# microsoft/hyperspace

Hardware: AMD Instinct MI355X
Metric: index-build GB/s + indexed filter/join query latency (s), 1/2/4/8 MI355X (higher is better)
Workload: dtype int64/fp64 columnar; 1 GPU; model=covering-index(key,val) build + filter + co-bucketed join, num_buckets=200, parallelism=bucket-parallel dp1, RCCL all-to-all exchange, device=cuda

## Files before the change

hyperspace_amd/csrc/binding.cpp:

```cpp

#include <torch/extension.h>

#include <c10/hip/HIPStream.h>

#include <algorithm>
#include <tuple>
#include <vector>

#include "kernels/kernels.h"

namespace {

hipStream_t current_stream() {
  return c10::hip::getCurrentHIPStream().stream();
}

void check_cuda(const torch::Tensor& t, const char* name) {
  TORCH_CHECK(t.is_cuda(), name, " must be a device tensor");
  TORCH_CHECK(t.is_contiguous(), name, " must be contiguous");
}

int normalize_dtype_code(torch::ScalarType t) {
  switch (t) {
    case torch::kInt64: return 0;
    case torch::kInt32: return 1;
    case torch::kFloat64: return 2;
    case torch::kFloat32: return 3;
    case torch::kInt16: return 4;
    case torch::kInt8: return 5;
    case torch::kBool: return 6;
    default:
      TORCH_CHECK(false, "unsupported sort-key dtype");
  }
}

torch::Tensor murmur3_bucket(std::vector<torch::Tensor> keys,
                             int64_t num_buckets,
                             std::vector<torch::Tensor> masks = {}) {
  TORCH_CHECK(!keys.empty(), "need at least one key column");
  TORCH_CHECK(masks.empty() || masks.size() == keys.size(),
              "masks must be empty or parallel to keys");
  TORCH_CHECK(num_buckets > 0 && num_buckets <= (int64_t)INT32_MAX,
              "murmur3_bucket: num_buckets must be in 1..INT32_MAX, got ",
              num_buckets);
  auto n = keys[0].numel();
  auto dev = keys[0].device();
  torch::Tensor h;
  if (keys.size() > 1)
    h = torch::empty({n}, torch::dtype(torch::kInt32).device(dev));
  auto out = torch::empty({n}, torch::dtype(torch::kInt32).device(dev));
  auto stream = current_stream();
  bool first = true;
  for (size_t ci = 0; ci < keys.size(); ++ci) {
    auto& k = keys[ci];
    check_cuda(k, "key");
    TORCH_CHECK(k.numel() == n, "key column length mismatch");
    torch::Tensor col = k;
    int kind;
    switch (col.scalar_type()) {
      case torch::kInt64:
        kind = 1;
        break;
      case torch::kFloat64:
        kind = 3;
        break;
      case torch::kInt32:
        kind = 0;
        break;
      case torch::kFloat32:
        kind = 2;
        break;
      case torch::kInt16:
      case torch::kInt8:
      case torch::kBool:
        col = col.to(torch::kInt32);
        kind = 0;
        break;
      default:
        TORCH_CHECK(false, "unsupported hash-key dtype");
    }
    const uint8_t* valid = nullptr;
    torch::Tensor mcol;
    if (!masks.empty() && masks[ci].numel() > 0) {
      mcol = masks[ci];
      check_cuda(mcol, "mask");
      TORCH_CHECK(mcol.numel() == n, "mask length mismatch");
      TORCH_CHECK(mcol.scalar_type() == torch::kBool ||
                      mcol.scalar_type() == torch::kUInt8,
                  "mask must be bool/uint8");
      valid = (const uint8_t*)mcol.data_ptr();
    }
// ... 659 lines not shown
                      masks[c].scalar_type() == torch::kUInt8,
                  "mask must be bool/uint8");
      held.push_back(aligned16(masks[c]));
      mptr[c] = (const uint8_t*)held.back().data_ptr();
    }
  }
  auto stream = current_stream();
  int64_t tile = hsk::group_tile_size();
  int64_t n_tiles = (n + tile - 1) / tile;
  auto tile_counts = torch::empty({n_tiles}, opts);
  hsk::group_offsets_count(kptr, mptr, (int)keys.size(), n,
                           tile_counts.data_ptr<int64_t>(), stream);
  auto tile_offsets = torch::empty({n_tiles}, opts);
  auto total = torch::empty({1}, opts);
  hsk::exclusive_scan_i64(tile_counts.data_ptr<int64_t>(),
                          tile_offsets.data_ptr<int64_t>(), n_tiles,
                          total.data_ptr<int64_t>(), stream);
  int64_t n_groups = total.cpu().item<int64_t>();
  auto out = torch::empty({n_groups + 1}, opts);
  hsk::group_offsets_emit(kptr, mptr, (int)keys.size(), n,
                          tile_offsets.data_ptr<int64_t>(),
                          total.data_ptr<int64_t>(), out.data_ptr<int64_t>(),
                          stream);
  return out;
}

std::vector<torch::Tensor> segmented_reduce(torch::Tensor values,
                                            torch::Tensor valid,
                                            torch::Tensor offsets,
                                            int64_t want) {
  check_cuda(values, "values");
  int dtype;
  switch (values.scalar_type()) {
    case torch::kInt64: dtype = 0; break;
    case torch::kInt32: dtype = 1; break;
    case torch::kFloat64: dtype = 2; break;
    case torch::kFloat32: dtype = 3; break;
    default:
      TORCH_CHECK(false, "segmented_reduce: values must be int32, int64, "
                         "float32 or float64");
  }
  bool is_float = dtype >= 2;
  auto dev = values.device();
  int64_t n = values.numel();
  auto off_d = offsets.to(dev, torch::kInt64).contiguous();
  TORCH_CHECK(off_d.numel() >= 1, "offsets must have n_groups + 1 entries");
  int64_t n_groups = off_d.numel() - 1;
  auto i64 = torch::dtype(torch::kInt64).device(dev);
  auto sum_opts = is_float ? torch::dtype(torch::kFloat64).device(dev) : i64;
  auto sums = torch::zeros({(want & 1) ? n_groups : 0}, sum_opts);
  auto mins = torch::zeros({(want & 2) ? n_groups : 0}, values.options());
  auto maxs = torch::zeros({(want & 4) ? n_groups : 0}, values.options());
  auto counts = torch::zeros({n_groups}, i64);
  if (n == 0 || n_groups == 0) return {sums, mins, maxs, counts};
  values = aligned16(values);
  const uint8_t* vptr = nullptr;
  if (valid.numel() > 0) {
    check_cuda(valid, "valid");
    TORCH_CHECK(valid.numel() == n, "valid length mismatch");
    TORCH_CHECK(valid.scalar_type() == torch::kBool ||
                    valid.scalar_type() == torch::kUInt8,
                "valid must be bool/uint8");
    valid = aligned16(valid);
    vptr = (const uint8_t*)valid.data_ptr();
  }
  int64_t tile = hsk::group_tile_size();
  int64_t n_tiles = (n + tile - 1) / tile;
  auto tile_groups = torch::empty({n_tiles + 1}, i64);
  auto partials =
      torch::empty({4 * hsk::segmented_reduce_num_blocks(n)}, i64);
  hsk::segmented_reduce(values.data_ptr(), dtype, vptr,
                        off_d.data_ptr<int64_t>(), n, n_groups,
                        (want & 1) ? sums.data_ptr() : nullptr,
                        (want & 2) ? mins.data_ptr() : nullptr,
                        (want & 4) ? maxs.data_ptr() : nullptr,
                        counts.data_ptr<int64_t>(),
                        tile_groups.data_ptr<int64_t>(),
                        partials.data_ptr<int64_t>(), current_stream());
  return {sums, mins, maxs, counts};
}

int64_t group_tile_size() { return hsk::group_tile_size(); }

}

torch::Tensor select_range_u64_pub(torch::Tensor keys, int64_t lo,
                                   int64_t hi, bool lo_incl, bool hi_incl) {
  TORCH_CHECK(keys.is_cuda() && keys.is_contiguous(), "keys");
  auto n = keys.numel();
  auto opts = torch::dtype(torch::kInt64).device(keys.device());
  if (n == 0) return torch::empty({0}, opts);
  auto stream = c10::hip::getCurrentHIPStream().stream();
  int64_t nb = hsk::select_num_blocks(n);
  auto bcounts = torch::empty({nb}, opts);
  auto total = torch::empty({1}, opts);
  uint64_t ulo = (uint64_t)lo;
  uint64_t uhi = (uint64_t)hi;
  hsk::select_range_count((const uint64_t*)keys.data_ptr<int64_t>(), n, ulo,
                          uhi, lo_incl, hi_incl,
                          bcounts.data_ptr<int64_t>(),
                          total.data_ptr<int64_t>(), stream);
  int64_t n_out = total.cpu().item<int64_t>();
  auto out = torch::empty({n_out}, opts);
  if (n_out > 0) {
    hsk::select_range_emit((const uint64_t*)keys.data_ptr<int64_t>(), n, ulo,
                           uhi, lo_incl, hi_incl,
                           bcounts.data_ptr<int64_t>(),
                           out.data_ptr<int64_t>(), stream);
  }
  return out;
}

PYBIND11_MODULE(TORCH_EXTENSION_NAME, m) {
  m.def("murmur3_bucket", &murmur3_bucket, "Spark-compatible murmur3 bucket",
        py::arg("keys"), py::arg("num_buckets"),
        py::arg("masks") = std::vector<torch::Tensor>{});
  m.def("normalize_key", &normalize_key, "order-preserving u64 key",
        py::arg("vals"), py::arg("canonical") = false);
  m.def("radix_sort_pairs", &radix_sort_pairs, "stable LSD radix sort");
  m.def("radix_sort_plan", &radix_sort_plan,
        "pass plan of the radix sort for a varying-bit mask: "
        "(radix, [shifts])");
  m.def("exclusive_scan", &exclusive_scan,
        "device-wide exclusive scan of an int64 tensor: (out, total)");
  m.def("merge_join", &merge_join, "segmented sorted merge join",
        py::arg("lkeys"), py::arg("rkeys"), py::arg("lseg"), py::arg("rseg"),
        py::arg("mode") = 0);
  m.def("select_range_u64", &select_range_u64_pub, "range filter compaction");
  m.def("isin_sorted", &isin_sorted, "sorted-set membership");
  m.def("segmented_minmax", &segmented_minmax, "per-segment min/max");
  m.def("bloom_build", &bloom_build, "bloom filter build");
  m.def("bloom_probe", &bloom_probe, "bloom filter probe");
  m.def("bloom_probe_many", &bloom_probe_many,
        "K9 device sketch-predicate probe over per-file filters");
  m.def("zorder_key", &zorder_key, "z-order bit interleave");
  m.def("gather_rows", &gather_rows,
        "row gather by an int64 or int32 index");
  m.def("bucket_sort_perm", &bucket_sort_perm,
        "fused (bucket, integer key) sort: (perm int32, sorted key column, "
        "seg) or None when the key range is too wide");
  m.def("copy_unaligned", &copy_unaligned,
        "device parquet page decode (unaligned copy)");
  m.def("run_merge_perm", &run_merge_perm,
        "segmented two-sorted-run merge permutation");
  m.def("group_offsets", &group_offsets,
        "offsets of adjacent equal-key runs: int64 [n_groups + 1]",
        py::arg("keys"), py::arg("masks") = std::vector<torch::Tensor>{});
  m.def("segmented_reduce", &segmented_reduce,
        "fused per-group (sum, min, max, count); want bits 1/2/4");
  m.def("group_tile_size", &group_tile_size,
        "rows per tile of the group-by kernels");
  m.def("snappy_decompress", &snappy_decompress,
        "device snappy raw-block page decompression; returns status");
  m.def("decode_def_levels", &decode_def_levels,
        "host RLE-hybrid def-level decode -> bool validity");
  m.def("parse_rle_runs_batch", &parse_rle_runs_batch,
        py::call_guard<py::gil_scoped_release>(),
        "batched RLE-hybrid run parse over many pages");
  m.def("parse_rle_runs", &parse_rle_runs,
        py::call_guard<py::gil_scoped_release>(),
        "host parse of an RLE/bit-packed hybrid run table");
  m.def("parse_byte_arrays", &parse_byte_arrays,
        py::call_guard<py::gil_scoped_release>(),
        "host PLAIN byte-array page parse -> (offsets, bytes)");
  m.def("host_memcpy", &host_memcpy,
        "GIL-released buffer -> cpu-u8-tensor memcpy");
  m.def("rle_decode", &rle_decode,
        "device RLE/bit-packed dictionary-index decode");
}
```

hyperspace_amd/index/covering/index.py:

```python

from __future__ import annotations

import os
from typing import Any, Dict, List, Optional, Tuple

import torch

from ..base import Index, IndexerContext
from ...config import IndexConstants
from ...exceptions import HyperspaceException
from ...log.entry import (Schema, register_derived_dataset,
                          COVERING_INDEX_TYPE)
from ... import ops
from ...execution.columnar import ColumnBatch, StringColumn
from ...sources.parquet_io import (bucket_file_name, write_batch_parquet,
                                   read_files_batch, bucket_id_of_file)


class CoveringIndex(Index):
    def __init__(self, indexed_columns: List[str],
                 included_columns: List[str], schema: Schema,
                 num_buckets: int, properties: Dict[str, str]):
        self.indexed_columns = list(indexed_columns)
        self.included_columns = list(included_columns)
        self.schema = schema
        self.num_buckets = num_buckets
        self._properties = dict(properties)

    @property
    def kind(self) -> str:
        return "CoveringIndex"

    @property
    def kind_abbr(self) -> str:
        return "CI"

    def indexed_columns_list(self) -> List[str]:
        return list(self.indexed_columns)

    def referenced_columns(self) -> List[str]:
        return self.indexed_columns + self.included_columns

    @property
    def can_handle_deleted_files(self) -> bool:
        return (self._properties.get(IndexConstants.LINEAGE_PROPERTY, "false")
                .lower() == "true")

    @property
    def has_lineage(self) -> bool:
        return self.can_handle_deleted_files

    def with_new_properties(self, props: Dict[str, str]) -> "CoveringIndex":
        return CoveringIndex(self.indexed_columns, self.included_columns,
                             self.schema, self.num_buckets, props)

    def to_json(self) -> Dict[str, Any]:
        return {
            "type": COVERING_INDEX_TYPE,
            "indexedColumns": self.indexed_columns,
            "includedColumns": self.included_columns,
            "schema": self.schema.to_json(),
            "numBuckets": self.num_buckets,
            "properties": self._properties,
        }

    @staticmethod
    def from_json(d: Dict[str, Any]) -> "CoveringIndex":
        return CoveringIndex(
            d["indexedColumns"], d["includedColumns"],
            Schema.from_json(d["schema"]), d["numBuckets"],
            d.get("properties", {}))

    def write(self, ctx: IndexerContext, index_data) -> List[str]:
        from ...execution.scan_stream import ScanStream
        os.makedirs(ctx.index_data_path, exist_ok=True)

        import torch.distributed as dist
        distributed = dist.is_available() and dist.is_initialized() and \
            dist.get_world_size() > 1
        task_id = dist.get_rank() if distributed else 0

        if isinstance(index_data, ScanStream):
            batches = index_data.batches()
            n_groups = len(index_data.file_groups())
        else:
# ... 253 lines not shown
                "includedColumns": self.included_columns,
                "numBuckets": self.num_buckets}



def _multi_key_sort_perm(batch: ColumnBatch, key_cols: List[str]
                         ) -> torch.Tensor:
    n = batch.num_rows
    dev = batch.device
    perm = torch.arange(n, dtype=torch.int64, device=dev)
    for c in reversed(key_cols):
        keys = ops.sql_key(batch.tensor(c))[perm]
        _, perm = ops.sort_pairs(keys, perm)
        m = batch.mask(c)
        if m is not None and not bool(m.all()):
            f = m[perm]
            perm = perm[torch.cat([
                torch.nonzero(~f, as_tuple=False).flatten(),
                torch.nonzero(f, as_tuple=False).flatten()])]
    return perm


def _bucket_seg_offsets(sorted_bkeys_u64: torch.Tensor, num_buckets: int
                        ) -> torch.Tensor:
    probes = ops.cpu_ref.normalize_key(
        torch.arange(num_buckets + 1, dtype=torch.int64)).to(
            sorted_bkeys_u64.device)
    if sorted_bkeys_u64.numel() and int(sorted_bkeys_u64.max()) >= 0 \
            and int(sorted_bkeys_u64.min()) >= 0:
        seg = torch.searchsorted(
            sorted_bkeys_u64,
            torch.arange(num_buckets + 1, dtype=torch.int64,
                         device=sorted_bkeys_u64.device))
        return seg.cpu()
    sortable = sorted_bkeys_u64 ^ (-0x8000000000000000)
    sortable_probes = probes ^ (-0x8000000000000000)
    return torch.searchsorted(sortable, sortable_probes).cpu()


def _fused_bucket_sort(batch: ColumnBatch, bucket_ids: torch.Tensor,
                       key_cols: List[str], num_buckets: int
                       ) -> Optional[Tuple[ColumnBatch, torch.Tensor]]:
    if len(key_cols) != 1 or os.environ.get("HS_FUSED_BUCKET_SORT") == "0":
        return None
    key_name = batch._stored_key(key_cols[0])
    key = batch.columns[key_name]
    if isinstance(key, StringColumn) or batch.has_nulls(key_name):
        return None
    res = ops.bucket_sort_perm(key, bucket_ids, num_buckets)
    if res is None:
        return None
    perm, sorted_key, seg = res
    cols: Dict[str, Any] = {}
    for k, v in batch.columns.items():
        if k == key_name:
            cols[k] = sorted_key
        elif isinstance(v, StringColumn):
            cols[k] = StringColumn(ops.gather_rows(v.codes, perm), v.values)
        else:
            cols[k] = ops.gather_rows(v, perm)
    return ColumnBatch(
        cols, {k: m[perm] for k, m in batch.masks.items()}), seg


def sort_by_bucket_and_keys(batch: ColumnBatch, bucket_ids: torch.Tensor,
                            key_cols: List[str], num_buckets: int
                            ) -> Tuple[ColumnBatch, torch.Tensor]:
    fused = _fused_bucket_sort(batch, bucket_ids, key_cols, num_buckets)
    if fused is not None:
        return fused
    perm = _multi_key_sort_perm(batch, key_cols)
    b64 = ops.gather_rows(bucket_ids.to(torch.int64), perm)
    sorted_bkeys, perm2 = ops.sort_pairs(ops.normalize_key(b64), perm)
    batch = batch.gather(perm2)
    probes = ops.cpu_ref.normalize_key(
        torch.arange(num_buckets + 1, dtype=torch.int64)).to(
            sorted_bkeys.device)
    sortable = sorted_bkeys ^ (-0x8000000000000000)
    sortable_probes = probes ^ (-0x8000000000000000)
    seg = torch.searchsorted(sortable, sortable_probes).cpu()
    return batch, seg


def write_bucketed(batch: ColumnBatch, seg: torch.Tensor, out_dir: str,
                   num_buckets: int, task_id: int = 0,
                   after_event: Optional["torch.cuda.Event"] = None
                   ) -> List[str]:
    from concurrent.futures import ThreadPoolExecutor
    from ...execution.columnar import StringColumn
    from ...sources.parquet_io import _pinned_get, _pinned_put
    on_device = batch.device.type == "cuda"
    if on_device and os.environ.get("HS_WRITE_V2"):
        if after_event is not None:
            torch.cuda.current_stream().wait_event(after_event)
        host_cols = {}
        host_masks = {}
        held_bufs = []
        for name, col in batch.columns.items():
            if isinstance(col, StringColumn):
                host_cols[name] = col.to("cpu")
                continue
            nb = col.numel() * col.element_size()
            bufp = _pinned_get(nb)
            host = bufp[:nb].view(col.dtype)
            host.copy_(col, non_blocking=True)
            host_cols[name] = host
            held_bufs.append(bufp)
        for name, m in batch.masks.items():
            host_masks[name] = m.to("cpu")
        torch.cuda.current_stream().synchronize()
        host_batch = ColumnBatch(host_cols, host_masks)
        out = write_bucketed(host_batch, seg, out_dir, num_buckets,
                             task_id)
        for bufp in held_bufs:
            _pinned_put(bufp)
        return out
    jobs = []
    for b in range(num_buckets):
        lo, hi = int(seg[b]), int(seg[b + 1])
        if hi <= lo:
            continue
        jobs.append((b, lo, hi,
                     os.path.join(out_dir, bucket_file_name(task_id, b))))

    streams = ([torch.cuda.Stream(device=batch.device)
                for _ in range(min(8, max(1, len(jobs))))]
               if on_device else [])

    def write_one(job_i):
        b, lo, hi, out = jobs[job_i]
        piece = batch.slice(lo, hi)
        held = []
        if on_device:
            s = streams[job_i % len(streams)]
            if after_event is not None:
                s.wait_event(after_event)
            cols = {}
            masks = {}
            with torch.cuda.stream(s):
                for name, col in piece.columns.items():
                    if isinstance(col, StringColumn):
                        cols[name] = col.to("cpu")
                        continue
                    nb = col.numel() * col.element_size()
                    bufp = _pinned_get(nb)
                    host = bufp[:nb].view(col.dtype)
                    host.copy_(col, non_blocking=True)
                    cols[name] = host
                    held.append(bufp)
                for name, m in piece.masks.items():
                    masks[name] = m.to("cpu")
            s.synchronize()
            piece = ColumnBatch(cols, masks)
        write_batch_parquet(piece, out)
        for bufp in held:
            _pinned_put(bufp)
        return out

    if len(jobs) <= 2:
        return [write_one(i) for i in range(len(jobs))]
    with ThreadPoolExecutor(max_workers=16) as pool:
        return list(pool.map(write_one, range(len(jobs))))


register_derived_dataset(COVERING_INDEX_TYPE, CoveringIndex)
```

hyperspace_amd/rules/score_optimizer.py:

```python

from __future__ import annotations

from typing import Dict, List, Tuple

from .candidate_collector import Candidate
from .filter_reason import ReasonCollector
from .hyperspace_rules import (AggregateIndexRule, FilterIndexRule,
                               HyperspaceRule, JoinIndexRule, NoOpRule)
from ..plan.nodes import LogicalPlan


class ScoreBasedIndexPlanOptimizer:
    def __init__(self, session, reasons: ReasonCollector):
        self.session = session
        self.reasons = reasons
        self.rules: List[HyperspaceRule] = [
            FilterIndexRule(session, reasons),
            JoinIndexRule(session, reasons),
            AggregateIndexRule(session, reasons),
        ]
        try:
            from ..index.zorder.rule import ZOrderFilterIndexRule
            self.rules.append(ZOrderFilterIndexRule(session, reasons))
        except ImportError:
            pass
        try:
            from ..index.dataskipping.rule import ApplyDataSkippingIndex
            self.rules.append(ApplyDataSkippingIndex(session, reasons))
        except ImportError:
            pass
        self.rules.append(NoOpRule(session, reasons))

    def apply(self, plan: LogicalPlan,
              candidates: Dict[int, List[Candidate]]) -> LogicalPlan:
        best, _ = self._rec_apply(plan, candidates, {})
        return best

    def _rec_apply(self, plan: LogicalPlan, candidates,
                   memo: Dict[int, Tuple[LogicalPlan, float]]
                   ) -> Tuple[LogicalPlan, float]:
        key = id(plan)
        if key in memo:
            return memo[key]
        best_plan, best_score = plan, -1.0
        for rule in self.rules:
            transformed, score = rule.apply(plan, candidates)
            if transformed is plan and rule.name != "NoOpRule" and \
                    score == 0.0:
                continue
            child_results = [self._rec_apply(c, candidates, memo)
                             for c in transformed.children]
            total = score + sum(s for _, s in child_results)
            if transformed is not plan or rule.name == "NoOpRule":
                candidate_plan = (
                    transformed.with_children([p for p, _ in child_results])
                    if child_results else transformed)
                if total > best_score:
                    best_plan, best_score = candidate_plan, total
        memo[key] = (best_plan, max(best_score, 0.0))
        return memo[key]
```

hyperspace_amd/sources/native_parquet.py:

```python

from __future__ import annotations

import os
import struct
from typing import Any, Dict, List, NamedTuple, Optional, Tuple

import numpy as np

MAGIC = b"PAR1"

T_INT32, T_INT64, T_FLOAT, T_DOUBLE, T_BYTE_ARRAY = 1, 2, 4, 5, 6
_NP_TO_PARQUET = {
    np.dtype("int64"): T_INT64,
    np.dtype("int32"): T_INT32,
    np.dtype("float64"): T_DOUBLE,
    np.dtype("float32"): T_FLOAT,
}
_PARQUET_TO_NP = {v: k for k, v in _NP_TO_PARQUET.items()}

ENC_PLAIN = 0
ENC_PLAIN_DICTIONARY = 2
ENC_RLE = 3
ENC_RLE_DICTIONARY = 8
CODEC_UNCOMPRESSED = 0
# ... 170 lines not shown
    w.field_i32(2, nbytes)
    w.field_i32(3, nbytes)
    w.field_struct_begin(5)
    w.field_i32(1, num_values)
    w.field_i32(2, encoding)
    w.field_i32(3, ENC_RLE if has_def_levels else ENC_PLAIN)
    w.field_i32(4, ENC_PLAIN)
    w.struct_end()
    w.struct_end()
    return bytes(w.buf)


def _dict_page_header(num_values: int, nbytes: int) -> bytes:
    w = TWriter()
    w.struct_begin()
    w.field_i32(1, PAGE_DICTIONARY)
    w.field_i32(2, nbytes)
    w.field_i32(3, nbytes)
    w.field_struct_begin(7)
    w.field_i32(1, num_values)
    w.field_i32(2, ENC_PLAIN_DICTIONARY)
    w.struct_end()
    w.struct_end()
    return bytes(w.buf)


def _bitpack(vals: np.ndarray, width: int) -> bytes:
    n = len(vals)
    pad = (-n) % 8
    if pad:
        vals = np.concatenate(
            [vals, np.zeros(pad, dtype=vals.dtype)])
    bits = ((vals[:, None].astype(np.uint64)
             >> np.arange(width, dtype=np.uint64)) & 1).astype(np.uint8)
    return np.packbits(bits.reshape(-1), bitorder="little").tobytes()


def _dict_indices_payload(codes: np.ndarray, num_dict: int) -> Tuple[
        bytes, int]:
    bw = max(1, (num_dict - 1).bit_length()) if num_dict > 1 else 1
    groups = (len(codes) + 7) // 8
    body = _varint((groups << 1) | 1) + _bitpack(codes, bw)
    return bytes([bw]) + body, bw


def _plain_byte_array_dict(values: List[str]) -> bytes:
    out = bytearray()
    for v in values:
        b = v.encode("utf-8")
        out += struct.pack("<I", len(b))
        out += b
    return bytes(out)


def _statistics(arr: np.ndarray) -> Tuple[bytes, bytes]:
    return arr.min().tobytes(), arr.max().tobytes()


def _def_levels_payload(mask: np.ndarray) -> bytes:
    groups = (len(mask) + 7) // 8
    packed = np.packbits(mask.astype(np.uint8), bitorder="little")
    body = _varint((groups << 1) | 1) + packed.tobytes()
    return struct.pack("<I", len(body)) + body


_LAYOUT_CACHE: "Dict[str, Tuple[Tuple[int, int], int, list]]" = {}
_LAYOUT_CACHE_MAX = 16384


def layout_cache_get(path: str):
    ent = _LAYOUT_CACHE.get(path)
    if ent is None:
        return None
    try:
        st = os.stat(path)
    except OSError:
        return None
    if ent[0] != (st.st_size, st.st_mtime_ns):
        _LAYOUT_CACHE.pop(path, None)
        return None
    return ent[1], ent[2]


def _layout_cache_put(path: str, num_rows: int, layouts: list) -> None:
    if len(_LAYOUT_CACHE) >= _LAYOUT_CACHE_MAX:
        for k in list(_LAYOUT_CACHE)[:_LAYOUT_CACHE_MAX // 8]:
            _LAYOUT_CACHE.pop(k, None)
    st = os.stat(path)
    _LAYOUT_CACHE[path] = ((st.st_size, st.st_mtime_ns), num_rows, layouts)


def write_parquet_native(columns: "Dict[str, np.ndarray]", path: str,
                         masks: "Optional[Dict[str, np.ndarray]]" = None
                         ) -> Tuple[int, int]:
    names = list(columns.keys())
    arrays: List[Any] = []
    for n in names:
        c = columns[n]
        arrays.append(c if isinstance(c, StrCol)
                      else np.ascontiguousarray(c))
    num_rows = len(arrays[0]) if arrays else 0
    col_masks: List[Optional[np.ndarray]] = []
    for n, a in zip(names, arrays):
        if not isinstance(a, StrCol) and a.dtype not in _NP_TO_PARQUET:
            raise ValueError(f"dtype {a.dtype} not supported natively")
        assert len(a) == num_rows
        m = (masks or {}).get(n)
        if m is not None and bool(m.all()):
            m = None
        col_masks.append(m)

    chunks: List[Any] = []
    col_meta: List[Tuple] = []
    layouts: List[ColumnChunkLayout] = []
    offset = 4
    for name, arr, mask in zip(names, arrays, col_masks):
        if isinstance(arr, StrCol):
            dict_payload = _plain_byte_array_dict(arr.values)
            dict_header = _dict_page_header(len(arr.values),
                                            len(dict_payload))
            dict_off = offset
            offset += len(dict_header) + len(dict_payload)
            chunks.append(dict_header)
            chunks.append(dict_payload)

            codes = arr.codes if mask is None else arr.codes[mask]
            null_count = int(num_rows - len(codes))
            idx_payload, bw = _dict_indices_payload(codes,
                                                    len(arr.values))
            lvl_len = 0
            if mask is None:
                payload: Any = idx_payload
            else:
                levels = _def_levels_payload(mask)
                lvl_len = len(levels)
                payload = levels + idx_payload
            header = _page_header(num_rows, len(payload), mask is not None,
                                  encoding=ENC_PLAIN_DICTIONARY)
            col_meta.append((name, T_BYTE_ARRAY, offset,
                             offset - dict_off + len(header) + len(payload),
                             num_rows, b"", b"", null_count,
                             mask is not None, dict_off))
            layouts.append(ColumnChunkLayout(
                name, np.dtype("int32"),
                [Page("dict", offset + len(header) + lvl_len + 1,
                      offset + len(header) + len(payload), num_rows, bw)],
                num_rows, "dict",
                DictPage(dict_off + len(dict_header), offset,
                         len(arr.values)), [mask],
                is_string=True, str_values=list(arr.values)))
            chunks.append(header)
            chunks.append(payload)
            offset += len(header) + len(payload)
            continue
        lvl_len = 0
        if mask is None:
            payload = arr.data.cast("B")
            null_count = 0
            valid = arr
        else:
            valid = arr[mask]
            levels = _def_levels_payload(mask)
            lvl_len = len(levels)
            payload = levels + valid.tobytes()
            null_count = int(num_rows - len(valid))
        nbytes = len(payload)
        header = _page_header(num_rows, nbytes, mask is not None)
        mn, mx = _statistics(valid) if len(valid) else (b"", b"")
        col_meta.append((name, _NP_TO_PARQUET[arr.dtype], offset,
                         len(header) + nbytes, num_rows, mn, mx,
                         null_count, mask is not None, None))
        layouts.append(ColumnChunkLayout(
# ... 631 lines not shown
```

setup.py:

```python

import os

from setuptools import setup

os.environ.setdefault("PYTORCH_ROCM_ARCH", "gfx950")

from torch.utils.cpp_extension import BuildExtension, CUDAExtension

ROOT = os.path.dirname(os.path.abspath(__file__))

setup(
    name="hyperspace_amd",
    version="0.1.0",
    description="MI355X-native covering-index acceleration engine",
    packages=["hyperspace_amd"],
    ext_modules=[
        CUDAExtension(
            name="hyperspace_amd._hip",
            sources=[
                "hyperspace_amd/csrc/binding.cpp",
                "hyperspace_amd/csrc/kernels/kernels.hip",
                "hyperspace_amd/csrc/kernels/aggregate.hip",
            ],
            include_dirs=[os.path.join(ROOT, "hyperspace_amd", "csrc")],
            extra_compile_args={
                "cxx": ["-O3", "-std=c++17"],
                "nvcc": ["-O3", "-std=c++17"],
            },
        )
    ],
    cmdclass={"build_ext": BuildExtension},
)
```

Measured before the change: 16.66 GB/s.

## Write bucket files natively via chunked D2H pinned ring and threaded pwrite

Adds a C++ bucket writer that streams device columns in chunks through a pinned host ring on two HIP streams. A pool of writer threads pwrites each chunk straight to its offset in the parquet file, and the footer is encoded in C++. Per-bucket min/max statistics are computed on the device with segmented_reduce, and the file layout cache is filled from the fstat results, so there is no extra os.stat per file. The aim is to overlap device-to-host copies with file I/O and to drop the per-file Python write overhead. In exchange it adds a large native code path with its own parquet encoding, threading and error handling, and it removes the HS_WRITE_V2 path.

```diff
diff --git a/hyperspace_amd/csrc/binding.cpp b/hyperspace_amd/csrc/binding.cpp
--- a/hyperspace_amd/csrc/binding.cpp
+++ b/hyperspace_amd/csrc/binding.cpp
@@ -4,9 +4,11 @@
 #include <c10/hip/HIPStream.h>
 
 #include <algorithm>
+#include <string>
 #include <tuple>
 #include <vector>
 
+#include "bucket_writer.h"
 #include "kernels/kernels.h"
 
 namespace {
@@ -832,6 +834,107 @@
 
 int64_t group_tile_size() { return hsk::group_tile_size(); }
 
+std::tuple<std::vector<int64_t>, std::vector<int64_t>, std::vector<int64_t>,
+           std::vector<int64_t>>
+write_bucket_files(std::vector<torch::Tensor> cols,
+                   std::vector<std::string> names,
+                   std::vector<std::string> paths,
+                   std::vector<int64_t> row_lo, std::vector<int64_t> row_hi,
+                   std::vector<std::string> mins,
+                   std::vector<std::string> maxs, torch::Tensor ring,
+                   int64_t chunk_bytes, int64_t writer_threads,
+                   int64_t stream0, int64_t stream1, bool timing) {
+  TORCH_CHECK(!cols.empty() && cols.size() == names.size(),
+              "write_bucket_files: columns and names must be parallel");
+  TORCH_CHECK(paths.size() == row_lo.size() && paths.size() == row_hi.size(),
+              "write_bucket_files: paths and row ranges must be parallel");
+  TORCH_CHECK(mins.size() == paths.size() * cols.size() &&
+                  maxs.size() == mins.size(),
+              "write_bucket_files: one (min, max) per file and column");
+  TORCH_CHECK(chunk_bytes > 0 && writer_threads >= 1 && writer_threads <= 15,
+              "write_bucket_files: chunk_bytes > 0, 1 <= threads <= 15");
+  const bool on_device = cols[0].is_cuda();
+  const int64_t n = cols[0].numel();
+  std::vector<hsw::Column> wc;
+  for (size_t c = 0; c < cols.size(); c++) {
+    const torch::Tensor& t = cols[c];
+    TORCH_CHECK(t.dim() == 1 && t.is_contiguous() && t.numel() == n &&
+                    t.device() == cols[0].device(),
+                "write_bucket_files: columns must be 1-D, contiguous, of "
+                "one length and on one device");
+    int ptype;
+    switch (t.scalar_type()) {
+      case torch::kInt64: ptype = hsw::T_INT64; break;
+      case torch::kInt32: ptype = hsw::T_INT32; break;
+      case torch::kFloat64: ptype = hsw::T_DOUBLE; break;
+      case torch::kFloat32: ptype = hsw::T_FLOAT; break;
+      default:
+        TORCH_CHECK(false, "write_bucket_files: unsupported column dtype");
+    }
+    wc.push_back({t.data_ptr(), (int)t.element_size(), ptype, names[c]});
+  }
+  std::vector<hsw::FileJob> jobs;
+  for (size_t f = 0; f < paths.size(); f++) {
+    TORCH_CHECK(0 <= row_lo[f] && row_lo[f] < row_hi[f] && row_hi[f] <= n,
+                "write_bucket_files: row range of file ", f,
+                " is empty or outside the batch");
+    jobs.push_back({paths[f], row_lo[f], row_hi[f]});
+  }
+  std::vector<std::pair<std::string, std::string>> stats;
+  for (size_t i = 0; i < mins.size(); i++)
+    stats.emplace_back(std::move(mins[i]), std::move(maxs[i]));
+
+  hsw::Options opt;
+  opt.chunk_bytes = (size_t)chunk_bytes;
+  opt.writer_threads = (int)writer_threads;
+  opt.device_source = on_device;
+  opt.timing = timing;
+  std::vector<hsw::FileResult> res;
+  if (on_device) {
+    TORCH_CHECK(ring.device().is_cpu() && ring.is_pinned() &&
+                    ring.is_contiguous() &&
+                    ring.scalar_type() == torch::kUInt8 &&
+                    ring.numel() >= chunk_bytes,
+                "write_bucket_files: ring must be a pinned uint8 tensor of "
+                "at least one chunk");
+    opt.streams[0] = reinterpret_cast<hipStream_t>(stream0);
+    opt.streams[1] = reinterpret_cast<hipStream_t>(stream1);
+    opt.ring = ring.data_ptr();
+    opt.ring_bytes = (size_t)ring.numel();
+    hipEvent_t start = nullptr;
+    TORCH_CHECK(hipEventCreateWithFlags(&start, hipEventDisableTiming) ==
+                    hipSuccess,
+                "write_bucket_files: hipEventCreate failed");
+    hipError_t e = hipEventRecord(start, current_stream());
+    opt.start_event = start;
+    std::string err;
+    if (e != hipSuccess) {
+      err = std::string("hipEventRecord: ") + hipGetErrorString(e);
+    } else {
+      py::gil_scoped_release rel;
+      try {
+        res = hsw::write_bucket_files(wc, jobs, stats, opt);
+      } catch (const std::exception& ex) {
+        err = ex.what();
+      }
+    }
+    (void)hipEventDestroy(start);
+    TORCH_CHECK(err.empty(), err);
+  } else {
+    py::gil_scoped_release rel;
+    res = hsw::write_bucket_files(wc, jobs, stats, opt);
+  }
+  std::vector<int64_t> sizes, mtimes, starts, ends;
+  for (const hsw::FileResult& r : res) {
+    sizes.push_back(r.size);
+    mtimes.push_back(r.mtime_ns);
+    starts.insert(starts.end(), r.payload_start.begin(),
+                  r.payload_start.end());
+    ends.insert(ends.end(), r.payload_end.begin(), r.payload_end.end());
+  }
+  return {sizes, mtimes, starts, ends};
+}
+
 }
 
 torch::Tensor select_range_u64_pub(torch::Tensor keys, int64_t lo,
@@ -898,6 +1001,9 @@
         py::arg("keys"), py::arg("masks") = std::vector<torch::Tensor>{});
   m.def("segmented_reduce", &segmented_reduce,
         "fused per-group (sum, min, max, count); want bits 1/2/4");
+  m.def("write_bucket_files", &write_bucket_files,
+        "write every bucket file of a batch: chunked D2H through a pinned "
+        "ring into pwrite (host batches: pwrite from the columns)");
   m.def("group_tile_size", &group_tile_size,
         "rows per tile of the group-by kernels");
   m.def("snappy_decompress", &snappy_decompress,
diff --git a/hyperspace_amd/csrc/bucket_writer.cpp b/hyperspace_amd/csrc/bucket_writer.cpp
--- /dev/null
+++ b/hyperspace_amd/csrc/bucket_writer.cpp
@@ -0,0 +1,533 @@
+
+#include "bucket_writer.h"
+
+#include <fcntl.h>
+#include <sys/stat.h>
+#include <unistd.h>
+
+#include <algorithm>
+#include <atomic>
+#include <cerrno>
+#include <chrono>
+#include <condition_variable>
+#include <cstdio>
+#include <cstring>
+#include <deque>
+#include <memory>
+#include <mutex>
+#include <stdexcept>
+#include <thread>
+
+namespace hsw {
+namespace {
+
+enum : int { CT_I32 = 5, CT_I64 = 6, CT_BINARY = 8, CT_LIST = 9,
+             CT_STRUCT = 12 };
+
+class TWriter {
+ public:
+  std::string buf;
+
+  void struct_begin() { last_.push_back(0); }
+  void struct_end() {
+    buf.push_back('\0');
+    last_.pop_back();
+  }
+  void field_i32(int fid, int64_t v) {
+    field(fid, CT_I32);
+    varint(zigzag(v));
+  }
+  void field_i64(int fid, int64_t v) {
+    field(fid, CT_I64);
+    varint(zigzag(v));
+  }
+  void field_binary(int fid, const std::string& s) {
+    field(fid, CT_BINARY);
+    binary(s);
+  }
+  void field_list_begin(int fid, int etype, size_t size) {
+    field(fid, CT_LIST);
+    if (size < 15) {
+      buf.push_back((char)((size << 4) | etype));
+    } else {
+      buf.push_back((char)(0xF0 | etype));
+      varint(size);
+    }
+  }
+  void field_struct_begin(int fid) {
+    field(fid, CT_STRUCT);
+    struct_begin();
+  }
+  void i32_elem(int64_t v) { varint(zigzag(v)); }
+  void binary(const std::string& s) {
+    varint(s.size());
+    buf += s;
+  }
+
+ private:
+  std::vector<int> last_{0};
+
+  static uint64_t zigzag(int64_t n) {
+    return ((uint64_t)n << 1) ^ (uint64_t)(n >> 63);
+  }
+  void varint(uint64_t n) {
+    while (true) {
+      uint8_t b = n & 0x7F;
+      n >>= 7;
+      if (n) {
+        buf.push_back((char)(b | 0x80));
+      } else {
+        buf.push_back((char)b);
+        return;
+      }
+    }
+  }
+  void field(int fid, int ctype) {
+    int delta = fid - last_.back();
+    if (delta > 0 && delta <= 15) {
+      buf.push_back((char)((delta << 4) | ctype));
+    } else {
+      buf.push_back((char)ctype);
+      varint(zigzag(fid));
+    }
+    last_.back() = fid;
+  }
+};
+
+struct ColMeta {
+  int64_t off;
+  int64_t nbytes;
+};
+
+std::string footer_bytes(const std::vector<Column>& cols,
+                         const std::vector<ColMeta>& meta, int64_t num_rows,
+                         const std::pair<std::string, std::string>* stats) {
+  TWriter w;
+  w.struct_begin();
+  w.field_i32(1, 2);
+  w.field_list_begin(2, CT_STRUCT, 1 + cols.size());
+  w.struct_begin();
+  w.field_binary(4, "schema");
+  w.field_i32(5, (int64_t)cols.size());
+  w.struct_end();
+  for (const Column& c : cols) {
+    w.struct_begin();
+    w.field_i32(1, c.ptype);
+    w.field_i32(3, 0);
+    w.field_binary(4, c.name);
+    w.struct_end();
+  }
+  w.field_i64(3, num_rows);
+  w.field_list_begin(4, CT_STRUCT, 1);
+  w.struct_begin();
+  int64_t total_bytes = 0;
+  w.field_list_begin(1, CT_STRUCT, cols.size());
+  for (size_t c = 0; c < cols.size(); c++) {
+    total_bytes += meta[c].nbytes;
+    const std::string& mn = stats[c].first;
+    const std::string& mx = stats[c].second;
+    w.struct_begin();
+    w.field_i64(2, meta[c].off);
+    w.field_struct_begin(3);
+    w.field_i32(1, cols[c].ptype);
+    w.field_list_begin(2, CT_I32, 1);
+    w.i32_elem(0);
+    w.field_list_begin(3, CT_BINARY, 1);
+    w.binary(cols[c].name);
+    w.field_i32(4, 0);
+    w.field_i64(5, num_rows);
+    w.field_i64(6, meta[c].nbytes);
+    w.field_i64(7, meta[c].nbytes);
+    w.field_i64(9, meta[c].off);
+    if (!mn.empty()) {
+      w.field_struct_begin(12);
+      w.field_binary(1, mx);
+      w.field_binary(2, mn);
+      w.field_i64(3, 0);
+      w.field_binary(5, mx);
+      w.field_binary(6, mn);
+      w.struct_end();
+    }
+    w.struct_end();
+    w.struct_end();
+  }
+  w.field_i64(2, total_bytes);
+  w.field_i64(3, num_rows);
+  w.struct_end();
+  w.field_binary(6, "hyperspace_amd 0.1");
+  w.struct_end();
+  return std::move(w.buf);
+}
+
+struct FilePlan {
+  std::vector<std::pair<int64_t, std::string>> pieces;
+  std::mutex open_mu;
+  bool open_tried = false;
+  int fd = -1;
+  std::atomic<int64_t> remaining{0};
+};
+
+struct Task {
+  int file;
+  int64_t file_off;
+  const char* src;
+  size_t nbytes;
+};
+
+constexpr size_t kFileGroup = 16;
+
+int64_t now_ns() {
+  return std::chrono::duration_cast<std::chrono::nanoseconds>(
+             std::chrono::steady_clock::now().time_since_epoch())
+      .count();
+}
+
+struct Issued {
+  size_t task;
+  int slot;
+};
+
+class Run {
+ public:
+  Run(const std::vector<FileJob>& files, const Options& opt,
+      std::vector<FileResult>& results)
+      : files_(files), opt_(opt), results_(results),
+        plans_(new FilePlan[files.size()]) {}
+
+  FilePlan* plans() { return plans_.get(); }
+  std::vector<Task> tasks;
+
+  void fail(const std::string& what) {
+    std::lock_guard<std::mutex> g(err_mu_);
+    if (!failed_.load()) {
+      error_ = what;
+      failed_.store(true);
+    }
+  }
+  bool failed() const { return failed_.load(); }
+  const std::string& error() const { return error_; }
+
+  void host_writer() {
+    while (!failed()) {
+      size_t i = next_.fetch_add(1);
+      if (i >= tasks.size()) return;
+      const int64_t t0 = now_ns();
+      write_task(tasks[i], tasks[i].src);
+      ns_write_ += now_ns() - t0;
+    }
+  }
+
+  void init_ring(int nslots, hipEvent_t* events) {
+    events_ = events;
+    for (int s = nslots - 1; s >= 0; s--) free_.push_back(s);
+  }
+
+  void copier() {
+    for (int s = 0; s < 2 && !failed(); s++)
+      hip(hipStreamWaitEvent(opt_.streams[s], opt_.start_event, 0),
+          "hipStreamWaitEvent");
+    for (size_t i = 0; i < tasks.size() && !failed(); i++) {
+      int slot;
+      {
+        const int64_t t0 = now_ns();
+        std::unique_lock<std::mutex> g(mu_);
+        cv_free_.wait(g, [&] { return !free_.empty(); });
+        slot = free_.back();
+        free_.pop_back();
+        ns_slot_wait_ += now_ns() - t0;
+      }
+      hipStream_t st = opt_.streams[i & 1];
+      char* dst = (char*)opt_.ring + (size_t)slot * opt_.chunk_bytes;
+      bool ok = !failed() &&
+                hip(hipMemcpyAsync(dst, tasks[i].src, tasks[i].nbytes,
+                                   hipMemcpyDeviceToHost, st),
+                    "hipMemcpyAsync");
+      if (ok && !hip(hipEventRecord(events_[slot], st), "hipEventRecord")) {
+        (void)hipStreamSynchronize(st);
+        ok = false;
+      }
+      std::lock_guard<std::mutex> g(mu_);
+      if (ok) {
+        issued_.push_back({i, slot});
+        cv_issued_.notify_one();
+      } else {
+        free_.push_back(slot);
+        break;
+      }
+    }
+    std::lock_guard<std::mutex> g(mu_);
+    copier_done_ = true;
+    cv_issued_.notify_all();
+  }
+
+  void ring_writer(int device) {
+    (void)hipSetDevice(device);
+    while (true) {
+      Issued it;
+      {
+        std::unique_lock<std::mutex> g(mu_);
+        cv_issued_.wait(g, [&] { return !issued_.empty() || copier_done_; });
+        if (issued_.empty()) return;
+        it = issued_.front();
+        issued_.pop_front();
+      }
+      const int64_t t0 = now_ns();
+      bool ok = hip(hipEventSynchronize(events_[it.slot]),
+                    "hipEventSynchronize");
+      const int64_t t1 = now_ns();
+      if (ok && !failed())
+        write_task(tasks[it.task], (const char*)opt_.ring +
+                                       (size_t)it.slot * opt_.chunk_bytes);
+      ns_event_wait_ += t1 - t0;
+      ns_write_ += now_ns() - t1;
+      std::lock_guard<std::mutex> g(mu_);
+      free_.push_back(it.slot);
+      cv_free_.notify_one();
+    }
+  }
+
+  void report(int64_t wall_ns, int nthreads) const {
+    std::fprintf(stderr,
+                 "[hs-timing] bucket writer: %zu chunks, wall %.3fs, copier "
+                 "waited for a free slot %.3fs; %d writers summed: copy "
+                 "wait %.3fs, open+pwrite+close %.3fs\n",
+                 tasks.size(), wall_ns * 1e-9, ns_slot_wait_.load() * 1e-9,
+                 nthreads, ns_event_wait_.load() * 1e-9,
+                 ns_write_.load() * 1e-9);
+  }
+
+  void close_all() {
+    for (size_t f = 0; f < files_.size(); f++) {
+      if (plans_[f].fd >= 0) {
+        ::close(plans_[f].fd);
+        plans_[f].fd = -1;
+      }
+    }
+  }
+
+ private:
+  const std::vector<FileJob>& files_;
+  const Options& opt_;
+  std::vector<FileResult>& results_;
+  std::unique_ptr<FilePlan[]> plans_;
+
+  std::atomic<bool> failed_{false};
+  std::mutex err_mu_;
+  std::string error_;
+  std::atomic<size_t> next_{0};
+  std::atomic<int64_t> ns_slot_wait_{0}, ns_event_wait_{0}, ns_write_{0};
+
+  std::mutex mu_;
+  std::condition_variable cv_free_, cv_issued_;
+  std::vector<int> free_;
+  std::deque<Issued> issued_;
+  bool copier_done_ = false;
+  hipEvent_t* events_ = nullptr;
+
+  bool hip(hipError_t e, const char* what) {
+    if (e == hipSuccess) return true;
+    fail(std::string(what) + ": " + hipGetErrorString(e));
+    return false;
+  }
+
+  void fail_io(const char* what, const std::string& path) {
+    fail(std::string(what) + " " + path + ": " + std::strerror(errno));
+  }
+
+  bool pwrite_all(int fd, const char* p, size_t n, int64_t off,
+                  const std::string& path) {
+    while (n) {
+      ssize_t w = ::pwrite(fd, p, n, (off_t)off);
+      if (w < 0) {
+        if (errno == EINTR) continue;
+        fail_io("pwrite", path);
+        return false;
+      }
+      p += w;
+      n -= (size_t)w;
+      off += w;
+    }
+    return true;
+  }
+
+  int ensure_open(int f) {
+    FilePlan& fp = plans_[f];
+    std::lock_guard<std::mutex> g(fp.open_mu);
+    if (!fp.open_tried) {
+      fp.open_tried = true;
+      const std::string& path = files_[f].path;
+      int fd = ::open(path.c_str(), O_WRONLY | O_CREAT | O_TRUNC | O_CLOEXEC,
+                      0666);
+      if (fd < 0) {
+        fail_io("open", path);
+        return -1;
+      }
+      fp.fd = fd;
+      for (const auto& pc : fp.pieces)
+        if (!pwrite_all(fd, pc.second.data(), pc.second.size(), pc.first,
+                        path))
+          break;
+    }
+    return failed() ? -1 : fp.fd;
+  }
+
+  void write_task(const Task& t, const char* src) {
+    int fd = ensure_open(t.file);
+    if (fd < 0) return;
+    const std::string& path = files_[t.file].path;
+    if (!pwrite_all(fd, src, t.nbytes, t.file_off, path)) return;
+    FilePlan& fp = plans_[t.file];
+    if (fp.remaining.fetch_sub(1, std::memory_order_acq_rel) != 1) return;
+    struct stat st;
+    if (::fstat(fd, &st) != 0) {
+      fail_io("fstat", path);
+      return;
+    }
+    results_[t.file].size = (int64_t)st.st_size;
+    results_[t.file].mtime_ns =
+        (int64_t)st.st_mtim.tv_sec * 1000000000LL + st.st_mtim.tv_nsec;
+    fp.fd = -1;
+    if (::close(fd) != 0) fail_io("close", path);
+  }
+};
+
+}
+
+std::string page_header_bytes(int64_t num_values, int64_t nbytes) {
+  TWriter w;
+  w.struct_begin();
+  w.field_i32(1, 0);
+  w.field_i32(2, nbytes);
+  w.field_i32(3, nbytes);
+  w.field_struct_begin(5);
+  w.field_i32(1, num_values);
+  w.field_i32(2, 0);
+  w.field_i32(3, 0);
+  w.field_i32(4, 0);
+  w.struct_end();
+  w.struct_end();
+  return std::move(w.buf);
+}
+
+std::vector<FileResult> write_bucket_files(
+    const std::vector<Column>& cols, const std::vector<FileJob>& files,
+    const std::vector<std::pair<std::string, std::string>>& stats,
+    const Options& opt) {
+  const size_t ncols = cols.size(), nfiles = files.size();
+  if (stats.size() != nfiles * ncols)
+    throw std::invalid_argument("write_bucket_files: stats size mismatch");
+  if (opt.chunk_bytes == 0 || opt.writer_threads < 1 ||
+      opt.writer_threads > 15)
+    throw std::invalid_argument(
+        "write_bucket_files: chunk_bytes > 0 and 1 <= writer_threads <= 15");
+  int nslots = 0;
+  if (opt.device_source) {
+    nslots = (int)std::min<size_t>(opt.ring_bytes / opt.chunk_bytes, 4096);
+    if (opt.ring == nullptr || nslots < 1)
+      throw std::invalid_argument(
+          "write_bucket_files: the ring holds no chunk");
+  }
+  std::vector<FileResult> results(nfiles);
+  if (nfiles == 0 || ncols == 0) return results;
+
+  Run run(files, opt, results);
+  const std::string magic("PAR1", 4);
+  std::vector<std::vector<Task>> file_tasks(nfiles);
+  for (size_t f = 0; f < nfiles; f++) {
+    const FileJob& job = files[f];
+    if (job.row_lo < 0 || job.row_hi <= job.row_lo)
+      throw std::invalid_argument("write_bucket_files: empty row range");
+    const int64_t rows = job.row_hi - job.row_lo;
+    FilePlan& fp = run.plans()[f];
+    FileResult& res = results[f];
+    fp.pieces.emplace_back(0, magic);
+    std::vector<ColMeta> meta(ncols);
+    int64_t off = 4;
+    int64_t chunks = 0;
+    for (size_t c = 0; c < ncols; c++) {
+      const int64_t nbytes = rows * cols[c].elem_size;
+      std::string header = page_header_bytes(rows, nbytes);
+      meta[c] = {off, (int64_t)header.size() + nbytes};
+      const int64_t start = off + (int64_t)header.size();
+      res.payload_start.push_back(start);
+      res.payload_end.push_back(start + nbytes);
+      fp.pieces.emplace_back(off, std::move(header));
+      const char* src = (const char*)cols[c].base +
+                        job.row_lo * (int64_t)cols[c].elem_size;
+      for (int64_t done = 0; done < nbytes;) {
+        size_t n = (size_t)std::min<int64_t>(nbytes - done,
+                                             (int64_t)opt.chunk_bytes);
+        file_tasks[f].push_back({(int)f, start + done, src + done, n});
+        done += (int64_t)n;
+        chunks++;
+      }
+      off = start + nbytes;
+    }
+    std::string tail = footer_bytes(cols, meta, rows, &stats[f * ncols]);
+    const uint32_t flen = (uint32_t)tail.size();
+    char le[4] = {(char)(flen & 0xFF), (char)((flen >> 8) & 0xFF),
+                  (char)((flen >> 16) & 0xFF), (char)((flen >> 24) & 0xFF)};
+    tail.append(le, 4);
+    tail += magic;
+    fp.pieces.emplace_back(off, std::move(tail));
+    fp.remaining.store(chunks);
+  }
+  for (size_t g = 0; g < nfiles; g += kFileGroup) {
+    const size_t g_end = std::min(nfiles, g + kFileGroup);
+    for (size_t j = 0;; j++) {
+      bool any = false;
+      for (size_t f = g; f < g_end; f++) {
+        if (j < file_tasks[f].size()) {
+          run.tasks.push_back(file_tasks[f][j]);
+          any = true;
+        }
+      }
+      if (!any) break;
+    }
+  }
+  file_tasks.clear();
+
+  const int nthreads =
+      (int)std::min<size_t>((size_t)opt.writer_threads, run.tasks.size());
+  std::vector<std::thread> threads;
+  std::vector<hipEvent_t> events;
+  const int64_t t_start = now_ns();
+  if (opt.device_source) {
+    int device = 0;
+    hipError_t e = hipGetDevice(&device);
+    for (int s = 0; s < nslots && e == hipSuccess; s++) {
+      hipEvent_t ev = nullptr;
+      e = hipEventCreateWithFlags(
+          &ev, hipEventBlockingSync | hipEventDisableTiming);
+      if (e == hipSuccess) events.push_back(ev);
+    }
+    if (e != hipSuccess) {
+      run.fail(std::string("hipEventCreate: ") + hipGetErrorString(e));
+    } else {
+      run.init_ring(nslots, events.data());
+      try {
+        for (int t = 0; t < nthreads; t++)
+          threads.emplace_back([&run, device] { run.ring_writer(device); });
+      } catch (const std::exception& ex) {
+        run.fail(std::string("thread start: ") + ex.what());
+      }
+      run.copier();
+    }
+  } else {
+    try {
+      for (int t = 0; t < nthreads; t++)
+        threads.emplace_back([&run] { run.host_writer(); });
+    } catch (const std::exception& ex) {
+      run.fail(std::string("thread start: ") + ex.what());
+    }
+  }
+  for (std::thread& t : threads) t.join();
+  for (hipEvent_t ev : events) (void)hipEventDestroy(ev);
+  run.close_all();
+  if (opt.timing) run.report(now_ns() - t_start, nthreads);
+  if (run.failed())
+    throw std::runtime_error("write_bucket_files: " + run.error());
+  return results;
+}
+
+}
diff --git a/hyperspace_amd/csrc/bucket_writer.h b/hyperspace_amd/csrc/bucket_writer.h
--- /dev/null
+++ b/hyperspace_amd/csrc/bucket_writer.h
@@ -0,0 +1,50 @@
+#pragma once
+
+#include <hip/hip_runtime_api.h>
+
+#include <cstddef>
+#include <cstdint>
+#include <string>
+#include <vector>
+
+namespace hsw {
+
+enum : int { T_INT32 = 1, T_INT64 = 2, T_FLOAT = 4, T_DOUBLE = 5 };
+
+struct Column {
+  const void* base;
+  int elem_size;
+  int ptype;
+  std::string name;
+};
+
+struct FileJob {
+  std::string path;
+  int64_t row_lo, row_hi;
+};
+
+struct FileResult {
+  int64_t size = 0;
+  int64_t mtime_ns = 0;
+  std::vector<int64_t> payload_start, payload_end;
+};
+
+struct Options {
+  size_t chunk_bytes = 8u << 20;
+  int writer_threads = 15;
+  bool device_source = false;
+  bool timing = false;
+  void* ring = nullptr;
+  size_t ring_bytes = 0;
+  hipStream_t streams[2] = {nullptr, nullptr};
+  hipEvent_t start_event = nullptr;
+};
+
+std::vector<FileResult> write_bucket_files(
+    const std::vector<Column>& cols, const std::vector<FileJob>& files,
+    const std::vector<std::pair<std::string, std::string>>& stats,
+    const Options& opt);
+
+std::string page_header_bytes(int64_t num_values, int64_t nbytes);
+
+}
diff --git a/hyperspace_amd/index/covering/index.py b/hyperspace_amd/index/covering/index.py
--- a/hyperspace_amd/index/covering/index.py
+++ b/hyperspace_amd/index/covering/index.py
@@ -1,6 +1,7 @@
 
 from __future__ import annotations
 
+import contextlib
 import os
 from typing import Any, Dict, List, Optional, Tuple
 
@@ -420,6 +421,120 @@
     return batch, seg
 
 
+_NATIVE_WRITE_DTYPES = (torch.int64, torch.int32, torch.float64,
+                        torch.float32)
+_WRITE_RING_SLOTS = 64
+
+
+def _native_write_eligible(batch: ColumnBatch) -> bool:
+    if os.environ.get("HS_NATIVE_WRITE") == "0" or batch.masks:
+        return False
+    if not batch.columns or not ops.native.available():
+        return False
+    return all(not isinstance(c, StringColumn)
+               and c.dtype in _NATIVE_WRITE_DTYPES and c.dim() == 1
+               and c.device == batch.device
+               for c in batch.columns.values())
+
+
+def _device_stat_unusable(v) -> bool:
+    return v != v or v == 0
+
+
+def _bucket_statistics(batch: ColumnBatch, jobs) -> Tuple[list, list]:
+    from ...sources.native_parquet import _statistics
+    ncols = len(batch.columns)
+    mins = [b""] * (len(jobs) * ncols)
+    maxs = [b""] * (len(jobs) * ncols)
+    on_device = batch.device.type == "cuda"
+    offsets = torch.tensor([jobs[0][1]] + [j[2] for j in jobs],
+                           dtype=torch.int64)
+    for c, col in enumerate(batch.columns.values()):
+        mm = None
+        if on_device:
+            lo0, hi1 = jobs[0][1], jobs[-1][2]
+            red = ops.segmented_reduce(col[lo0:hi1], None, offsets - lo0,
+                                       want=("min", "max"))
+            mm = torch.stack([red["min"], red["max"]]).cpu().numpy()
+        for f, (_, lo, hi, _) in enumerate(jobs):
+            if mm is not None and not (
+                    col.dtype.is_floating_point
+                    and (_device_stat_unusable(mm[0, f])
+                         or _device_stat_unusable(mm[1, f]))):
+                mn, mx = mm[0, f].tobytes(), mm[1, f].tobytes()
+            else:
+                mn, mx = _statistics(col[lo:hi].cpu().numpy())
+            mins[f * ncols + c] = mn
+            maxs[f * ncols + c] = mx
+    return mins, maxs
+
+
+def _write_bucketed_native(batch: ColumnBatch, jobs,
+                           after_event: Optional["torch.cuda.Event"]
+                           ) -> List[str]:
+    import time as _time
+    import numpy as np
+    from ...sources.native_parquet import (ColumnChunkLayout, Page,
+                                           _layout_cache_put)
+    from ...sources.staging import _pinned_get, _pinned_put
+    timing = os.environ.get("HS_TIMING")
+    t0 = _time.perf_counter()
+    on_device = batch.device.type == "cuda"
+    names = list(batch.columns.keys())
+    cols = [c.contiguous() for c in batch.columns.values()]
+    chunk = max(1, int(float(os.environ.get("HS_WRITE_CHUNK_MB", "8"))
+                       * (1 << 20)))
+    threads = min(15, max(1, int(os.environ.get("HS_WRITE_THREADS", "15"))))
+    paths = [j[3] for j in jobs]
+    row_lo = [j[1] for j in jobs]
+    row_hi = [j[2] for j in jobs]
+    ring = None
+    streams = (0, 0)
+    if on_device:
+        if after_event is not None:
+            torch.cuda.current_stream(batch.device).wait_event(after_event)
+        esz = max(c.element_size() for c in cols)
+        largest = max(hi - lo for lo, hi in zip(row_lo, row_hi)) * esz
+        chunk = min(chunk, -(-largest // 4096) * 4096)
+        n_chunks = sum(-(-(hi - lo) * c.element_size() // chunk)
+                       for lo, hi in zip(row_lo, row_hi) for c in cols)
+        ring = _pinned_get(chunk * max(2, min(_WRITE_RING_SLOTS, n_chunks)))
+    try:
+        with torch.cuda.device(batch.device) if on_device \
+                else contextlib.nullcontext():
+            mins, maxs = _bucket_statistics(batch, jobs)
+            t1 = _time.perf_counter()
+            if on_device:
+                pool = [torch.cuda.Stream(device=batch.device)
+                        for _ in range(2)]
+                streams = tuple(s.cuda_stream for s in pool)
+            sizes, mtimes, starts, ends = ops.native.ext().write_bucket_files(
+                cols, names, paths, row_lo, row_hi, mins, maxs,
+                ring if ring is not None
+                else torch.empty(0, dtype=torch.uint8),
+                chunk, threads, streams[0], streams[1], bool(timing))
+    finally:
+        if ring is not None:
+            _pinned_put(ring)
+    ncols = len(cols)
+    np_dtypes = [np.dtype(str(c.dtype).replace("torch.", "")) for c in cols]
+    for f, path in enumerate(paths):
+        rows = row_hi[f] - row_lo[f]
+        _layout_cache_put(path, rows, [
+            ColumnChunkLayout(
+                names[c], np_dtypes[c],
+                [Page("plain", starts[f * ncols + c], ends[f * ncols + c],
+                      rows)], rows, "plain", None, [None])
+            for c in range(ncols)], (sizes[f], mtimes[f]))
+    if timing:
+        import sys as _sys
+        t2 = _time.perf_counter()
+        print(f"[hs-timing] native write: stats {t1-t0:.3f}s "
+              f"files {t2-t1:.3f}s ({len(paths)} files, chunk {chunk} B, "
+              f"{threads} writers)", file=_sys.stderr)
+    return paths
+
+
 def write_bucketed(batch: ColumnBatch, seg: torch.Tensor, out_dir: str,
                    num_buckets: int, task_id: int = 0,
                    after_event: Optional["torch.cuda.Event"] = None
@@ -428,31 +543,6 @@
     from ...execution.columnar import StringColumn
     from ...sources.parquet_io import _pinned_get, _pinned_put
     on_device = batch.device.type == "cuda"
-    if on_device and os.environ.get("HS_WRITE_V2"):
-        if after_event is not None:
-            torch.cuda.current_stream().wait_event(after_event)
-        host_cols = {}
-        host_masks = {}
-        held_bufs = []
-        for name, col in batch.columns.items():
-            if isinstance(col, StringColumn):
-                host_cols[name] = col.to("cpu")
-                continue
-            nb = col.numel() * col.element_size()
-            bufp = _pinned_get(nb)
-            host = bufp[:nb].view(col.dtype)
-            host.copy_(col, non_blocking=True)
-            host_cols[name] = host
-            held_bufs.append(bufp)
-        for name, m in batch.masks.items():
-            host_masks[name] = m.to("cpu")
-        torch.cuda.current_stream().synchronize()
-        host_batch = ColumnBatch(host_cols, host_masks)
-        out = write_bucketed(host_batch, seg, out_dir, num_buckets,
-                             task_id)
-        for bufp in held_bufs:
-            _pinned_put(bufp)
-        return out
     jobs = []
     for b in range(num_buckets):
         lo, hi = int(seg[b]), int(seg[b + 1])
@@ -460,6 +550,9 @@
             continue
         jobs.append((b, lo, hi,
                      os.path.join(out_dir, bucket_file_name(task_id, b))))
+
+    if len(jobs) > 2 and _native_write_eligible(batch):
+        return _write_bucketed_native(batch, jobs, after_event)
 
     streams = ([torch.cuda.Stream(device=batch.device)
                 for _ in range(min(8, max(1, len(jobs))))]
diff --git a/hyperspace_amd/rules/score_optimizer.py b/hyperspace_amd/rules/score_optimizer.py
--- a/hyperspace_amd/rules/score_optimizer.py
+++ b/hyperspace_amd/rules/score_optimizer.py
@@ -37,11 +37,11 @@
         return best
 
     def _rec_apply(self, plan: LogicalPlan, candidates,
-                   memo: Dict[int, Tuple[LogicalPlan, float]]
+                   memo: Dict[int, tuple]
                    ) -> Tuple[LogicalPlan, float]:
         key = id(plan)
         if key in memo:
-            return memo[key]
+            return memo[key][:2]
         best_plan, best_score = plan, -1.0
         for rule in self.rules:
             transformed, score = rule.apply(plan, candidates)
@@ -57,5 +57,5 @@
                     if child_results else transformed)
                 if total > best_score:
                     best_plan, best_score = candidate_plan, total
-        memo[key] = (best_plan, max(best_score, 0.0))
-        return memo[key]
+        memo[key] = (best_plan, max(best_score, 0.0), plan)
+        return memo[key][:2]
diff --git a/hyperspace_amd/sources/native_parquet.py b/hyperspace_amd/sources/native_parquet.py
--- a/hyperspace_amd/sources/native_parquet.py
+++ b/hyperspace_amd/sources/native_parquet.py
@@ -276,12 +276,15 @@
     return ent[1], ent[2]
 
 
-def _layout_cache_put(path: str, num_rows: int, layouts: list) -> None:
+def _layout_cache_put(path: str, num_rows: int, layouts: list,
+                      stat: Optional[Tuple[int, int]] = None) -> None:
     if len(_LAYOUT_CACHE) >= _LAYOUT_CACHE_MAX:
         for k in list(_LAYOUT_CACHE)[:_LAYOUT_CACHE_MAX // 8]:
             _LAYOUT_CACHE.pop(k, None)
-    st = os.stat(path)
-    _LAYOUT_CACHE[path] = ((st.st_size, st.st_mtime_ns), num_rows, layouts)
+    if stat is None:
+        st = os.stat(path)
+        stat = (st.st_size, st.st_mtime_ns)
+    _LAYOUT_CACHE[path] = (tuple(stat), num_rows, layouts)
 
 
 def write_parquet_native(columns: "Dict[str, np.ndarray]", path: str,
diff --git a/setup.py b/setup.py
--- a/setup.py
+++ b/setup.py
@@ -19,6 +19,7 @@
             name="hyperspace_amd._hip",
             sources=[
                 "hyperspace_amd/csrc/binding.cpp",
+                "hyperspace_amd/csrc/bucket_writer.cpp",
                 "hyperspace_amd/csrc/kernels/kernels.hip",
                 "hyperspace_amd/csrc/kernels/aggregate.hip",
             ],
```

After: 18.17 GB/s, median of 6. 9.1% higher.
